# ziadabohalawa/6DoF-Pose-Estimation-and-Defect-Projection

Hardware: AMD Instinct MI355X
Metric: Mrays/s ray-mesh + ICP iters/s, 640x576 vs 100k-tri mesh (higher is better)
Workload: dtype f32 rays / f64 ICP (f32 MFMA filter)

## Files before the change

### 6dof-pose-estimation-and-defect-projection_amd/_lib.py

```python
import ctypes as C
import os
import sys
import threading

import numpy as np

_HERE = os.path.dirname(os.path.abspath(__file__))
LIB_PATH = os.environ.get("PEDP_LIB", os.path.join(_HERE, "libpedp_hip.so"))

HOST, DEVICE = 0, 1
POINT_TO_PLANE, POINT_TO_POINT = 0, 1


class PreprocessParams(C.Structure):
    _fields_ = [("voxel_size", C.c_double), ("plane_distance", C.c_double), ("plane_iterations", C.c_int32),
                ("first_frame", C.c_int32), ("seed", C.c_uint64), ("normal_radius", C.c_double), ("normal_max_nn", C.c_int32),
                ("cluster_min_points", C.c_int32), ("cluster_eps", C.c_double), ("outlier_neighbors", C.c_int32),
                ("flags", C.c_int32), ("outlier_std_ratio", C.c_double), ("average_normal_voxel", C.c_double)]

ALLREDUCE_FN = C.CFUNCTYPE(C.c_int, C.c_void_p, C.c_void_p, C.c_int, C.c_void_p)


class IcpParams(C.Structure):
    _fields_ = [
# ... 82 lines not shown
    "pedp_icp_batched": (C.c_int, [C.c_void_p, C.c_void_p, C.c_void_p, _P(IcpParams), C.c_void_p, C.c_int,
                                   C.c_void_p, C.c_void_p, C.c_void_p]),
    "pedp_icp_batched_ex": (C.c_int, [C.c_void_p, C.c_void_p, C.c_void_p, _P(IcpParams), C.c_void_p, C.c_int,
                                      C.c_void_p, C.c_void_p, C.c_void_p, C.c_void_p]),
    "pedp_nn": (C.c_int, [C.c_void_p, C.c_void_p, C.c_void_p, C.c_void_p, C.c_void_p, C.c_void_p]),
    "pedp_nn_last_sweep_ms": (C.c_int, [C.c_void_p, _P(C.c_float)]),
    "pedp_icp_last_stats": (C.c_int, [C.c_void_p, _P(C.c_int64), _P(C.c_int64), _P(C.c_int64)]),
    "pedp_icp_last_planned_passes": (C.c_int, [C.c_void_p, _P(C.c_int64)]),
    "pedp_icp_last_serial_path": (C.c_int, [C.c_void_p, _P(C.c_int64), _P(C.c_int64)]),
    "pedp_icp_last_head_closed": (C.c_int, [C.c_void_p, _P(C.c_int64), _P(C.c_int64), _P(C.c_int64)]),
    "pedp_icp_last_certified": (C.c_int, [C.c_void_p, _P(C.c_int64), _P(C.c_int64)]),
    "pedp_icp_last_steady": (C.c_int, [C.c_void_p, _P(C.c_int64), _P(C.c_int64)]),
    "pedp_icp_last_steady_followers": (C.c_int, [C.c_void_p, _P(C.c_int64)]),
    "pedp_icp_last_lane_solves": (C.c_int, [C.c_void_p, _P(C.c_int64)]),
    "pedp_debug_nn_bf16": (C.c_int, [C.c_void_p, C.c_void_p, C.c_int64, C.c_void_p, C.c_int64, C.c_void_p]),
    "pedp_debug_solve6": (C.c_int, [C.c_void_p, C.c_int64, C.c_void_p, C.c_void_p, C.c_void_p, C.c_void_p, C.c_void_p, C.c_void_p]),
    "pedp_debug_icp_path": (C.c_int, [C.c_void_p, C.c_void_p, C.c_void_p]),
    "pedp_icp_begin": (C.c_int, [C.c_void_p, C.c_void_p, C.c_void_p, _P(IcpParams), C.c_void_p, C.c_int]),
    "pedp_icp_end": (C.c_int, [C.c_void_p, C.c_void_p, _P(C.c_double), _P(C.c_double), _P(C.c_int32), C.c_void_p, C.c_void_p]),
    "pedp_icp_configure": (C.c_int, [C.c_void_p, C.c_int, C.c_int]),
    "pedp_comm_unique_id": (C.c_int, [C.c_void_p]),
    "pedp_comm_create": (C.c_int, [C.c_void_p, C.c_void_p, C.c_int, C.c_int]),
    "pedp_comm_destroy": (C.c_int, [C.c_void_p]),
    "pedp_comm_size": (C.c_int, [C.c_void_p, _P(C.c_int), _P(C.c_int)]),
    "pedp_comm_allgather": (C.c_int, [C.c_void_p, C.c_void_p, C.c_void_p, C.c_int64]),
    "pedp_comm_allreduce_f64": (C.c_int, [C.c_void_p, C.c_void_p, C.c_int64]),
    "pedp_render": (C.c_int, [C.c_void_p, C.c_void_p, C.c_int64, C.c_void_p, C.c_int64, C.c_void_p, C.c_void_p, C.c_void_p,
                              C.c_void_p, C.c_int, C.c_int, C.c_void_p, C.c_void_p, C.c_int, C.c_void_p, C.c_int, C.c_void_p,
                              C.c_void_p, C.c_void_p, C.c_void_p]),
    "pedp_rasterize": (C.c_int, [C.c_void_p, C.c_void_p, C.c_int, C.c_int64, C.c_void_p, C.c_int64, C.c_int, C.c_int, C.c_int,
# ... 718 lines not shown
    return a.value


def icp_last_lane_solves(ctx):
    a = C.c_int64(0)
    check(load().pedp_icp_last_lane_solves(ctx._h, C.byref(a)), "pedp_icp_last_lane_solves")
    return a.value


ICP_SWITCHES = ("nn_f32", "unfused_finish", "no_visit_plan", "serial_close", "copy_bracket", "head_close", "cert", "steady")
ICP_PATH_FIELDS = ("fused", "dev_result", "copy_bracket", "head", "certify", "plan", "serial_close", "unfused_finish", "exchange",
                   "steady", "steady_from")


class IcpSwitches(C.Structure):
    _fields_ = [(n, C.c_int) for n in ICP_SWITCHES + ("steady_from", "steady_grid", "target_order", "steady_closers", "steady_groups", "lane_solve")]


class IcpPathInputs(C.Structure):
    _fields_ = [("n_source", C.c_int64), ("n_target", C.c_int64), ("radius", C.c_double)] + [
        (n, C.c_int) for n in ("unit_size", "poses", "timed_pass", "exhaustive", "exchange", "batch", "early_exit", "no_steady", "resident")]


class IcpPath(C.Structure):
    _fields_ = [(n, C.c_int) for n in ICP_PATH_FIELDS + ("lane_solve",)]


def icp_path(switches=None, steady_from=5, n_source=1, n_target=1, radius=1.0, unit_size=1, poses=1, timed_pass=-1, lane_solve=None,
             **flags):
    sw = None
    if switches is not None:
# ... 98 lines not shown


def debug_solve6(ctx, A, b):
    A = np.ascontiguousarray(A, np.float64).reshape(-1, 36)
    b = np.ascontiguousarray(b, np.float64).reshape(-1, 6)
    n = len(A)
    if len(b) != n:
        raise ValueError("debug_solve6: A and b differ in their count")
    out = {"x_lanes": np.empty((n, 6), np.float64), "ok_lanes": np.empty(n, np.int32),
           "x_one": np.empty((n, 6), np.float64), "ok_one": np.empty(n, np.int32)}
    check(load().pedp_debug_solve6(ctx._h, n, _ptr(A), _ptr(b), _ptr(out["x_lanes"]), _ptr(out["ok_lanes"]), _ptr(out["x_one"]),
                                   _ptr(out["ok_one"])), "pedp_debug_solve6")
    return out


def icp_begin(ctx, source, target, max_correspondence_distance, init, estimator=POINT_TO_PLANE, max_iteration=30,
              relative_fitness=1e-6, relative_rmse=1e-6, want_trace=False, n_source_global=0, use_comm=False):
    prm = IcpParams()
    prm.max_correspondence_distance = float(max_correspondence_distance)
    prm.estimator = int(estimator)
    prm.max_iteration = int(max_iteration)
    prm.relative_fitness = float(relative_fitness)
    prm.relative_rmse = float(relative_rmse)
    prm.allreduce = C.cast(None, ALLREDUCE_FN)
    prm.allreduce_user = None
    prm.n_source_global = int(n_source_global)
    prm.use_comm = int(bool(use_comm))
    T0 = np.ascontiguousarray(init, dtype=np.float64).reshape(4, 4)
    check(load().pedp_icp_begin(ctx._h, source._h, target._h, C.byref(prm), _ptr(T0), 1 if want_trace else 0), "pedp_icp_begin")
    ctx._icp_pending = (source, target, int(max_iteration), bool(want_trace))
# ... 102 lines not shown
```

### 6dof-pose-estimation-and-defect-projection_amd/csrc/icp/fused_close.h

```cpp
#pragma once
#include "common.h"
#include "solve.h"
#include "solve_lanes.h"

namespace {

constexpr int CH = NN_SB * 16;
constexpr int BK_W = 8;
constexpr int BK_WCAP = BK_W * 64;
constexpr int PSTRIDE = 32;
constexpr int LIVE_CAP = 8192;
constexpr int FIN_THREADS = 1024;

__device__ __forceinline__ void swap_if(bool c, double &x, double &y) {
    const double t = x;
    x = c ? y : x;
    y = c ? t : y;
}
__device__ bool solve6_ldlt_reg(const double *__restrict__ Ain, const double *__restrict__ b, double *__restrict__ x) {
    double A[6][6], y[6];
    int tr[6];
#pragma unroll
    for (int i = 0; i < 6; ++i)
#pragma unroll
// ... 161 lines not shown
    int serial = 0;
    int lane = 0;
    unsigned long long *live_old = nullptr;
    int gen_masks = 0;
};
template <int NT, int LCAP>
struct FinishLds {
    double slice[32][32], pk[32];
    int scan[NT], lst[LCAP];
    int do_rebuild, n_live_s, stopped;
    double t0[16];
};
__device__ __forceinline__ double bcast0(double v) {
    return __hiloint2double(__builtin_amdgcn_readfirstlane(__double2hiint(v)), __builtin_amdgcn_readfirstlane(__double2loint(v)));
}
typedef __attribute__((address_space(1))) unsigned long long g_u64;
typedef __attribute__((address_space(1))) int g_i32;
typedef __attribute__((address_space(1))) unsigned g_u32;
__device__ __forceinline__ double load_sc1(const double *p) {
    return __longlong_as_double((long long)__hip_atomic_load((g_u64 *)(uintptr_t)p, __ATOMIC_RELAXED, __HIP_MEMORY_SCOPE_AGENT));
}
__device__ __forceinline__ int load_sc1(const int32_t *p) {
    return __hip_atomic_load((g_i32 *)(uintptr_t)p, __ATOMIC_RELAXED, __HIP_MEMORY_SCOPE_AGENT);
}
__device__ __forceinline__ void store_sc1(double *p, double v) {
    __hip_atomic_store((g_u64 *)(uintptr_t)p, (unsigned long long)__double_as_longlong(v), __ATOMIC_RELAXED, __HIP_MEMORY_SCOPE_AGENT);
}
template <bool COHERENT>
__device__ __forceinline__ double load_partial(const double *p) {
    return COHERENT ? load_sc1(p) : *p;
}
template <bool COHERENT>
__device__ __forceinline__ unsigned long long load_live(unsigned long long *p) {
    if (COHERENT) return __hip_atomic_fetch_or((g_u64 *)(uintptr_t)p, 0ull, __ATOMIC_RELAXED, __HIP_MEMORY_SCOPE_AGENT);
    return *p;
}

#define PEDP_STAMP_CLOSE(unit, slot) do { if (!HEAD || blockIdx.x == 0) PEDP_STAMP(2, unit, slot); } while (0)
template <int NT, int LCAP, bool COHERENT, int MODE = 0>
__device__ __forceinline__ void icp_finish_body(IcpState *st, const FinishArgs &f, FinishLds<NT, LCAP> &L, const int tid) {
    constexpr bool LOCAL = MODE != 0, HEAD = MODE >= 2;
    static_assert(MODE != 2 || !COHERENT, "the head close reads what the launch before stored");
    static_assert(MODE != 3 || COHERENT, "the close inside a steady launch reads what that launch stored");
    auto uni = [](double v) { return LOCAL ? bcast0(v) : v; };
    const int pass = f.known ? f.k_pass : st->pass, max_iter = LOCAL ? __builtin_amdgcn_readfirstlane(st->max_iter) : st->max_iter;
    const double n_source = uni(st->n_source), rel_fitness = uni(st->rel_fitness), rel_rmse = uni(st->rel_rmse), reachE = uni(st->reachE),
                 margin = uni(st->margin);
    constexpr int PARTS = 32, TPARTS = NT / 32, PPT = PARTS / TPARTS;
    static_assert(NT % 32 == 0 && PARTS % TPARTS == 0, "thread count");
    const bool wide = f.serial == 0;
    if (tid == 0) { L.do_rebuild = 0; L.stopped = 0; }
    if (tid == 0) PEDP_STAMP_CLOSE(0, 0);
    if (tid == 0 && pass == 5) PEDP_STAMP_CLOSE(3, 0);
    const bool early_look = wide && COHERENT && f.n_idle > 0;
    unsigned look0 = 0u, idle_base0 = 0u;
    if (early_look && tid < 64) {
        if (tid < 16) look0 = __hip_atomic_load((g_u32 *)(uintptr_t)(f.idle + 32 * tid), __ATOMIC_RELAXED, __HIP_MEMORY_SCOPE_AGENT);
        idle_base0 = st->idle_base;
    }
    double fit0 = 0.0, rmse0 = 0.0, mu_th0 = 0.0, mu_ta0 = 0.0;
    int n_wide0 = 0;
    if (tid < 16) L.t0[tid] = st->T[tid];
    if (tid == 0) {
        fit0 = st->fitness; rmse0 = st->rmse; mu_th0 = st->mu_theta; mu_ta0 = st->mu_tau;
        if (wide) n_wide0 = st->n_wide;
    }
#if PEDP_ICP_STAMPS
    if (tid == 0 && (!HEAD || blockIdx.x == 0)) { g_icp_stamps[2][1][0] = (long long)__builtin_amdgcn_s_memtime(); g_icp_stamps[2][1][1] = (long long)__builtin_amdgcn_s_memrealtime(); }
#endif
    if (f.phase != 2) {
        const bool listing = !HEAD && (f.known ? f.k_rebuild != 0 : st->rebuild != 0);
        int n_live = f.known ? f.k_n_live : st->n_live;
        bool listed = true;
        if (listing) {
            const int per = (f.n_lw + NT - 1) / NT;
            const int w_lo = tid * per < f.n_lw ? tid * per : f.n_lw, w_hi = w_lo + per < f.n_lw ? w_lo + per : f.n_lw;
            int mine = 0;
            unsigned long long first = 0ull;
            for (int wi = w_lo; wi < w_hi; ++wi) {
                const unsigned long long word = load_live<COHERENT>(&f.live[wi]);
                if (wi == w_lo) first = word;
                mine += __builtin_popcountll(word);
            }
            L.scan[tid] = mine;
            __syncthreads();
            for (int off = 1; off < NT; off <<= 1) {
                const int t = tid >= off ? L.scan[tid - off] : 0;
                __syncthreads();
                L.scan[tid] += t;
                __syncthreads();
            }
            n_live = L.scan[NT - 1];
            listed = n_live <= LCAP;
            int at = L.scan[tid] - mine;
            for (int wi = w_lo; wi < w_hi; ++wi) {
                unsigned long long word = wi == w_lo ? first : load_live<COHERENT>(&f.live[wi]);
                while (word != 0ull) {
                    const int chunk = wi * 64 + __builtin_ctzll(word);
                    word &= word - 1ull;
                    if (listed) L.lst[at] = chunk;
                    as_global(f.live_list)[at] = chunk;
                    ++at;
                }
            }
            __syncthreads();
        }
        const int k = tid & 31;
        const int lper = (n_live + PARTS - 1) / PARTS;
        auto sum_ranges = [&](auto position) {
            if constexpr (PPT == 2) {
                constexpr int BW = 10;
                const int part = tid >> 4, k0 = (tid & 15) * 2, k1 = k0 + 1;
                const bool has1 = k1 < PACKET + (LOCAL ? 3 : 2);
                const int l_lo = part * lper < n_live ? part * lper : n_live, l_hi = l_lo + lper < n_live ? l_lo + lper : n_live;
                double v0 = 0.0, v1 = 0.0;
                for (int q = l_lo; q < l_hi; q += BW) {
                    int at[BW];
                    double x0[BW], x1[BW];
#pragma unroll
                    for (int u = 0; u < BW; ++u) at[u] = position(q + u < l_hi ? q + u : l_hi - 1);
// ... 31 lines not shown
                        double x[BW1];
#pragma unroll
                        for (int u = 0; u < BW1; ++u) at[u] = position(q + u < l_hi ? q + u : l_hi - 1);
#pragma unroll
                        for (int u = 0; u < BW1; ++u) x[u] = load_partial<COHERENT>(&f.partials[(size_t)at[u] * PSTRIDE + k]);
#pragma unroll
                        for (int u = 0; u < BW1; ++u) v = q + u < l_hi ? v + x[u] : v;
                    }
                }
                L.slice[part][k] = v;
            }
        };
        if (!listing) sum_ranges([&](int q) { return q; });
        else if (listed) sum_ranges([&](int q) { return L.lst[q]; });
        else sum_ranges([&](int q) { return load_sc1(&f.live_list[q]); });
        if (tid == 0 && pass == 5) PEDP_STAMP_CLOSE(3, 1);
        if (HEAD) PEDP_RT(pass + 1, 5);
        if (tid == 0) L.n_live_s = n_live;
        __syncthreads();
        if (tid == 0 && pass == 5) PEDP_STAMP_CLOSE(3, 2);
        if (tid < 32) {
            double t = 0.0;
            for (int q = 0; q < PARTS; ++q) t += L.slice[q][tid];
            L.pk[tid] = t;
            if (!HEAD && tid < PACKET) as_global(f.packet)[tid] = t;
        }
        __syncthreads();
        if (HEAD) PEDP_RT(pass + 1, 6);
        if (tid == 0 && f.phase == 1) {
            st->sum_tiles += (long long)L.pk[PACKET];
            st->sum_fb += (long long)L.pk[PACKET + 1];
            st->n_live = L.n_live_s;
        }
        if (tid == 0) {
#if PEDP_ICP_STAMPS
// ... 27 lines not shown
                st->done = -1;
                if (!LOCAL && f.down) *(int *)((char *)f.down + offsetof(IcpState, done)) = -1;
            }
            return;
        }
    }
    if (wide ? tid < 64 : tid == 0) {
        const bool l0 = tid == 0;
        int stop_i = 0, angles_i = 0;
        int solve_i = 0;
        const bool lane_form = wide && f.lane != 0;
        double upd[16], x[6] = {0.0, 0.0, 0.0, 0.0, 0.0, 0.0};
        ident4(upd);
        if (l0) {
            PEDP_STAMP_CLOSE(0, 1);
            if (pass == 5) PEDP_STAMP_CLOSE(3, 3);
            if (COHERENT) { st->ticket_base += (unsigned)f.n_busy; st->idle_base += (unsigned)f.n_idle; }
            if (f.phase == 0) {
                st->sum_tiles += (long long)L.pk[PACKET];
                st->sum_fb += (long long)L.pk[PACKET + 1];
                st->n_live = L.n_live_s;
                if constexpr (LOCAL) {
                    const long long searched = (long long)(L.pk[PACKET + 2] / CERT_PACK);
                    st->sum_searched += searched;
                    st->sum_cert += (long long)(L.pk[PACKET + 2] - (double)searched * CERT_PACK);
                }
            }
            L.do_rebuild = 0;
            const double *pk = L.pk;
            const double K = pk[28];
            double fit = 0.0, rmse = 0.0;
// ... 9 lines not shown
            }
            st->iters = pass;
            if (wide) st->n_wide = n_wide0 + 1;
            if (HEAD) st->n_head = st->n_head + 1;
            bool stop = pass >= max_iter;
            if (pass > 0 && fabs(fit0 - fit) < rel_fitness && fabs(rmse0 - rmse) < rel_rmse) stop = true;
            if (stop) {
                st->done = 1;
                if (!LOCAL && COHERENT && f.down) {
                    L.stopped = 1;
                    asm volatile("s_waitcnt vmcnt(0)" ::: "memory");
                }
                stop_i = 1;
            } else {
                PEDP_STAMP_CLOSE(2, 0);
                if (pass == 5) PEDP_STAMP_CLOSE(3, 4);
                if (K > 0.0) {
                    if (f.estimator == PEDP_POINT_TO_PLANE && lane_form) {
                        solve_i = 1;
                    } else if (f.estimator == PEDP_POINT_TO_PLANE) {
                        double A[36], nb[6];
                        int k = 0;
#pragma unroll
                        for (int u = 0; u < 6; ++u)
#pragma unroll
                            for (int v = u; v < 6; ++v) { A[6 * u + v] = pk[k]; A[6 * v + u] = pk[k]; ++k; }
#pragma unroll
                        for (int u = 0; u < 6; ++u) nb[u] = -pk[21 + u];
                        const bool ok = solve6_ldlt_reg(A, nb, x);
                        PEDP_STAMP_CLOSE(2, 1);
                        if (ok) {
// ... 50 lines not shown
                    if (!lane_form) {
#pragma unroll
                        for (int k = 0; k < 6; ++k) x[k] = bcast0(x[k]);
                    }
                    double s, c;
                    sincos(tid == 0 ? x[0] : (tid == 1 ? x[1] : x[2]), &s, &c);
                    const double sa = __shfl(s, 0, 64), ca = __shfl(c, 0, 64), sb = __shfl(s, 1, 64), cb = __shfl(c, 1, 64),
                                 sc = __shfl(s, 2, 64), cc = __shfl(c, 2, 64);
                    sincos_to_T(sa, ca, sb, cb, sc, cc, x, upd);
                    if (l0) PEDP_STAMP_CLOSE(2, 2);
                } else {
#pragma unroll
                    for (int k = 0; k < 16; ++k) upd[k] = bcast0(upd[k]);
                }
                if (l0) PEDP_STAMP_CLOSE(0, 2);
                if (l0 && pass == 5) PEDP_STAMP_CLOSE(3, 5);
                const int i = (tid >> 2) & 3, j = tid & 3;
                double tn = 0.0, u_ij = 0.0;
#pragma unroll
                for (int k = 0; k < 4; ++k) {
                    const double a = i == 0 ? upd[k] : (i == 1 ? upd[4 + k] : (i == 2 ? upd[8 + k] : upd[12 + k]));
                    const double b = L.t0[4 * k + j];
                    tn += a * b;
                    u_ij = j == k ? a : u_ij;
                }
                if (tid < 16) {
                    st->upd[tid] = u_ij;
                    if (!HEAD) as_global(f.hist)[16 * (pass + 1) + tid] = u_ij;
                    st->T[tid] = tn;
                }
            } else {
                PEDP_STAMP_CLOSE(0, 2);
                if (pass == 5) PEDP_STAMP_CLOSE(3, 5);
                for (int k = 0; k < 16; ++k) { st->upd[k] = upd[k]; if (!HEAD) as_global(f.hist)[16 * (pass + 1) + k] = upd[k]; }
                double Tn[16];
                mat4_mul_dev(upd, L.t0, Tn);
                for (int k = 0; k < 16; ++k) st->T[k] = Tn[k];
            }
            if (l0) {
                double th2 = 0.0, tv[3];
                for (int u = 0; u < 3; ++u) {
                    tv[u] = upd[4 * u + 3];
                    const double cc[3] = {f.bcx, f.bcy, f.bcz};
                    for (int v = 0; v < 3; ++v) {
                        const double dlt = upd[4 * u + v] - (u == v ? 1.0 : 0.0);
                        th2 += dlt * dlt;
                        tv[u] += dlt * cc[v];
                    }
                }
                double mu_th = mu_th0 + sqrt(th2), mu_ta = mu_ta0 + sqrt(tv[0] * tv[0] + tv[1] * tv[1] + tv[2] * tv[2]);
                const double mu = mu_th * reachE + mu_ta;
                if (!(mu < 0.95 * margin)) {
                    L.do_rebuild = 1;
                    mu_th = 0.0;
                    mu_ta = 0.0;
                    st->n_rebuilds += 1;
                }
                st->mu_theta = mu_th;
                st->mu_tau = mu_ta;
                st->rebuild = L.do_rebuild;
                st->pass = pass + 1;
                PEDP_STAMP_CLOSE(2, 3);
                if (pass == 5) PEDP_STAMP_CLOSE(3, 6);
            }
        }
        if (l0) PEDP_STAMP_CLOSE(0, 3);
    }
    __syncthreads();
    if (!HEAD && !f.gen_masks && L.do_rebuild)
        for (int wi = tid; wi < f.n_lw; wi += NT) { as_global(f.live_old)[wi] = load_live<COHERENT>(&f.live[wi]); as_global(f.live)[wi] = 0ull; }
    if (!HEAD && f.gen_masks && f.known && f.k_rebuild)
        for (int wi = tid; wi < f.n_lw; wi += NT) as_global(f.live_old)[wi] = 0ull;
    if (!LOCAL && COHERENT && f.down && L.stopped)
        for (int i = tid; i < (int)(sizeof(IcpState) / sizeof(double)); i += NT) ((double *)f.down)[i] = load_sc1((const double *)st + i);
}

__global__ __launch_bounds__(FIN_THREADS) void icp_finish_kernel(IcpState *st, unsigned long long *live, int32_t *live_list,
                                                         int n_lw, const double *partials, double *packet, int phase, int estimator,
// ... 43 lines not shown
```

### 6dof-pose-estimation-and-defect-projection_amd/csrc/icp/fused_pass.h

```cpp
#pragma once
#include "fused_close.h"
#include "segmented_sweep.h"

namespace {

constexpr int WTL = 1024;
constexpr int L2_WORDS = 8;
constexpr int SW_G = 8;

__device__ __forceinline__ void scan_near_tiles(unsigned long long near, int unit_of_lane, const PassArgs &a, double qx,
                                                double qy, double qz, int lane, double &bd, int &bj) {
    while (near != 0ull) {
        int unit = -1;
#pragma unroll
        for (int g = 0; g < 4; ++g) {
            if (near != 0ull) {
                const int bit = __builtin_ctzll(near);
                near &= near - 1ull;
                const int u = __shfl(unit_of_lane, bit, 64);
                if (g == (lane >> 4)) unit = u;
            }
        }
        const int64_t row = (int64_t)unit * 16 + (lane & 15);
        if (unit >= 0 && row < a.Nt)
// ... 205 lines not shown
                                   __HIP_MEMORY_SCOPE_AGENT);
        return;
    }
#if PEDP_ICP_STAMPS
    if (threadIdx.x == 0 && pass < 32 && blockIdx.x < 512 && blockIdx.y == 0) g_icp_rt[pass][blockIdx.x][0] = rt_entry;
#endif
    PEDP_RT(pass, 1);
    const bool certify = !BATCH && a0.cert != nullptr;
    const float inf = __uint_as_float(0x7F800000u);
    const double dinf = __longlong_as_double(0x7FF0000000000000ll);
    const double dnan = __longlong_as_double(0x7FF8000000000000ll);
    const double ccx_b = BATCH ? st->centroid[0] : 0.0, ccy_b = BATCH ? st->centroid[1] : 0.0, ccz_b = BATCH ? st->centroid[2] : 0.0;
    const float r_search_b = BATCH ? st->r_search : 0.f;
#define PEDP_CC(k, b) (BATCH ? (b) : bcast0(cur.centroid[k]))
    unsigned long long todo = 0ull;
    int todo_base = -64, it = 0;
    if (rebuild && threadIdx.x == 0) {
        double Rs[12];
#pragma unroll
        for (int k = 0; k < 12; ++k) { Rs[k] = PEDP_ST.T[k]; rbs[k] = Rs[k]; }
        double m = 0.0;
#pragma unroll
        for (int u = 0; u < 3; ++u) {
            double row = 0.0;
#pragma unroll
            for (int v = 0; v < 3; ++v) row += fabs(Rs[u] * Rs[v] + Rs[4 + u] * Rs[4 + v] + Rs[8 + u] * Rs[8 + v]);
            m = row > m ? row : m;
        }
        rbs[12] = sqrt(m) * (1.0 + 1e-9);
        rbs[13] = sqrt(PEDP_ST.r2live) * (1.0 + 1e-9);
    }
    __syncthreads();
    for (;;) {
        int tid = threadIdx.x;
        asm volatile("" : "+v"(tid));
        const int lane = tid & 63, wv = __builtin_amdgcn_readfirstlane(tid >> 6);
        const int half = wv >> 2, q4 = wv & 3;
        const int j = lane & 15, g = lane >> 4;
        const int frag = j * 4 + g;
        const unsigned long long lt = (1ull << lane) - 1ull;
        const PEDP_GLOBAL double *Pk_in = as_global(a.Pk) + (size_t)(pass & 1) * a.pp_stride, *Tp_in = as_global(a.Tprev) + (size_t)(pass & 1) * a.pp_stride;
        PEDP_GLOBAL double *Pk_out = as_global(a.Pk) + (size_t)((pass + 1) & 1) * a.pp_stride, *Tp_out = as_global(a.Tprev) + (size_t)((pass + 1) & 1) * a.pp_stride;
        int chunk, unit;
        if (rebuild) {
            bool more = true;
            while (todo == 0ull) {
                todo_base += 64;
                if ((long long)blockIdx.x + (long long)todo_base * (long long)gdim >= (long long)a.n_chunks) { more = false; break; }
                const long long u = (long long)blockIdx.x + (long long)(todo_base + lane) * (long long)gdim;
                bool visit = false, withdraw = false;
                if (u < (long long)a.n_chunks) {
                    double Rs[12];
#pragma unroll
                    for (int k = 0; k < 12; ++k) Rs[k] = rbs[k];
                    const double rscale = rbs[12], reach = rbs[13];
                    const bool was_live = (as_global(PEDP_MASK_OLD)[u >> 6] >> (u & 63)) & 1ull;
#pragma unroll 2
                    for (int sb = 0; sb < 8; ++sb) {
                        const PEDP_GLOBAL double *sp8 = as_global(a.chunk_sph) + (size_t)(8 * u + sb) * 4;
                        const double cx = sp8[0], cy = sp8[1], cz = sp8[2], cr = sp8[3];
                        const double tx = Rs[0] * cx + Rs[1] * cy + Rs[2] * cz + Rs[3], ty = Rs[4] * cx + Rs[5] * cy + Rs[6] * cz + Rs[7],
                                     tz = Rs[8] * cx + Rs[9] * cy + Rs[10] * cz + Rs[11];
                        const double ex = fmax(fmax(a.lo[0] - tx, tx - a.hi[0]), 0.0), ey = fmax(fmax(a.lo[1] - ty, ty - a.hi[1]), 0.0),
                                     ez = fmax(fmax(a.lo[2] - tz, tz - a.hi[2]), 0.0);
                        const double lim = cr * rscale + reach + 1e-9 * (fabs(tx) + fabs(ty) + fabs(tz) + 1.0);
                        visit |= !(cr < 0.0) && !(ex * ex + ey * ey + ez * ez > lim * lim);
                    }
                    withdraw = !visit && (was_live || pass == 0);
                }
                todo = __builtin_amdgcn_ballot_w64(visit);
                unsigned long long wd = __builtin_amdgcn_ballot_w64(withdraw);
                while (wd != 0ull) {
                    const int i = __builtin_ctzll(wd);
                    wd &= wd - 1ull;
                    const int64_t k = ((int64_t)blockIdx.x + (int64_t)(todo_base + i) * gdim) * CH + tid;
                    if (tid < CH && k < a.N) as_global(a.idx_out)[as_global(a.perm)[k]] = -1;
                }
            }
            if (!more) break;
            const int i = __builtin_ctzll(todo);
            todo &= todo - 1ull;
            unit = (int)(blockIdx.x + (unsigned)(todo_base + i) * (unsigned)gdim);
            chunk = unit;
        } else {
            unit = (int)(blockIdx.x + (unsigned)it * (unsigned)gdim);
            ++it;
            if (unit >= n_live) break;
            if (planned && it == 1) { unit = vis[0]; chunk = vis[1]; }
            else chunk = unit == (int)blockIdx.x ? chunk_next : as_global(a.live_list)[unit];
        }
        long long t_chunk0 = 0;
        if (!BATCH && !rebuild) t_chunk0 = (long long)__builtin_amdgcn_s_memtime();
        if (tid == 0) PEDP_STAMP(1, blockIdx.x, 0);
        PEDP_WV(0, __builtin_amdgcn_s_memtime());
        PEDP_WV(9, pass);
        PEDP_WV(10, __builtin_amdgcn_s_memrealtime());
        PEDP_WV(12, ((long long)__builtin_amdgcn_s_getreg(63508) << 32) | (unsigned)__builtin_amdgcn_s_getreg(63492));
        int nsl;
        bool skip = false;
        {
            bool cand = false, near = false, certd = false;
            int pi = -1, jprev = -1;
            float c_new = 0.f;
            double x = 0.0, y = 0.0, z = 0.0, dprev = dnan, d2prev = dnan;
            const int64_t k = (int64_t)chunk * CH + half * 64 + lane;
            const bool valid = k < a.N;
            if (valid) {
                pi = as_global(a.perm)[k];
// ... 542 lines not shown
```

### 6dof-pose-estimation-and-defect-projection_amd/csrc/pedp_icp.hip

```cpp
#include "pedp_internal.h"
#include <atomic>
#include <cmath>
#include <cstddef>
#include <cstdlib>
#include <cstring>
#include <new>

#if defined(__HIP_DEVICE_COMPILE__) && !defined(__gfx950__)
#error "pedp_icp.hip: the fence-free close of a pass rests on gfx950's caches; build with --offload-arch=gfx950 only"
#endif

#include "icp/common.h"
#include "icp/prep.h"
#include "icp/target_order.h"
#include "icp/segmented_sweep.h"
#include "icp/segmented_select.h"
#include "icp/solve.h"
#include "icp/ransac.h"
#include "icp/fused_close.h"
#include "icp/fused_pass.h"
#include "icp/steady_pass.h"

namespace {

// ... 168 lines not shown
}

using IcpSwitches = pedp_icp_switches;
inline const IcpSwitches &icp_switches() {
    static const IcpSwitches sw = [] {
        auto flag = [](const char *name, int unset) { const char *v = getenv(name); return v ? atoi(v) != 0 : unset; };
        auto num = [](const char *name, int unset) { const char *v = getenv(name); return v && *v ? atoi(v) : unset; };
        const char *order = getenv("PEDP_ICP_TARGET_ORDER");
        IcpSwitches s;
        s.nn_f32 = flag("PEDP_NN_F32", 0); s.unfused_finish = flag("PEDP_ICP_UNFUSED_FINISH", 0);
        s.no_visit_plan = flag("PEDP_ICP_NO_VISIT_PLAN", 0); s.serial_close = flag("PEDP_ICP_SERIAL_CLOSE", 0);
        s.copy_bracket = flag("PEDP_ICP_COPY_BRACKET", 0); s.head_close = flag("PEDP_ICP_HEAD_CLOSE", 1);
        s.cert = flag("PEDP_ICP_CERT", 1); s.steady = flag("PEDP_ICP_STEADY", 1);
        s.steady_from = num("PEDP_ICP_STEADY_FROM", 5); s.steady_grid = num("PEDP_ICP_STEADY_GRID", 0);
        s.steady_closers = num("PEDP_ICP_STEADY_CLOSERS", 0); s.steady_groups = num("PEDP_ICP_STEADY_GROUPS", 0);
        s.lane_solve = num("PEDP_ICP_LANE_SOLVE", 1);
        s.target_order = order && !strcmp(order, "hilbert") ? PEDP_TARGET_ORDER_HILBERT
                         : order && !strcmp(order, "compact") ? PEDP_TARGET_ORDER_COMPACT : PEDP_TARGET_ORDER_AUTO;
        return s;
    }();
    return sw;
}

using IcpPath = pedp_icp_path;
using IcpPathInputs = pedp_icp_path_inputs;
inline bool fused_eligible(int qt, bool exhaustive, double r, int64_t Ns, int64_t Nt) {
    return qt == 1 && !exhaustive && r > 0.0 && Ns > 0 && Nt > 0 && (Nt + 1023) / 1024 <= BK_WCAP;
}
inline IcpPath icp_decide_path(const IcpSwitches &sw, const IcpPathInputs &in) {
    IcpPath p{};
    p.fused = fused_eligible(in.unit_size, in.exhaustive, in.radius, in.n_source, in.n_target);
// ... 136 lines not shown
    pa.cert = path.certify ? w.cert : nullptr; pa.cert_stride = (size_t)w.Ns_pad;
    pa.visit = path.plan ? w.visit : nullptr; pa.dur = path.plan ? w.dur : nullptr; pa.visit_cap = w.visit_cap; pa.n_cu = x->num_cus;
}

struct PassLaunch {
    int pass = 0;
    bool steady_launch = false;
    hipEvent_t ev0 = nullptr, ev1 = nullptr;
};

int enqueue_fused_pass(pedp_ctx_t c, const IcpJob &job, const PassLaunch &l) {
    PassArgs pa = job.pa;
    pa.launch = pa.head ? l.pass : 0;
    int64_t g = job.w.n_chunks;
    if (g > 2 * c->num_cus) g = 2 * c->num_cus;
    if (g < 1) g = 1;
    if (pa.head) g += 1;
    if (l.ev0) PEDP_HIP_CHECK(hipEventRecord(l.ev0, c->stream));
    if (l.steady_launch) {
        const int asked = icp_switches().steady_closers;
        const SteadyShape sh = steady_shape(c, job.w.n_chunks);
        double *const follow = job.w.follow_cap > 0 ? job.w.follow : nullptr;
        const int n_closers = asked > 0 ? asked : c->num_cus;
        auto steady = [&](auto kernel, int groups) {
            hipLaunchKernelGGL(kernel, dim3((unsigned)sh.grid), dim3(groups * BK_W * 64), 0, c->stream, job.w.st, pa, follow, job.w.follow_cap, n_closers);
        };
        if (sh.groups == 2) { if (pa.lane_solve) steady(icp_steady_kernel<2, true>, 2); else steady(icp_steady_kernel<2, false>, 2); }
        else { if (pa.lane_solve) steady(icp_steady_kernel<1, true>, 1); else steady(icp_steady_kernel<1, false>, 1); }
    } else {
        const bool batch = job.in.poses > 1;
// ... 927 lines not shown
        hipLaunchKernelGGL(solve6_lanes_debug_kernel, dim3((unsigned)((n + 3) / 4)), dim3(256), 0, c->stream, (const double *)d_A, (const double *)d_b, n, d_x, d_ok);
        hipLaunchKernelGGL(solve6_one_debug_kernel, dim3((unsigned)((n + 3) / 4)), dim3(256), 0, c->stream, (const double *)d_A, (const double *)d_b, n,
                           d_x + 6 * (size_t)n, d_ok + (size_t)n);
        e = hipGetLastError();
    }
    if (e == hipSuccess) e = hipMemcpyAsync(x_lanes, d_x, sizeof(double) * 6 * (size_t)n, hipMemcpyDeviceToHost, c->stream);
    if (e == hipSuccess) e = hipMemcpyAsync(x_one, d_x + 6 * (size_t)n, sizeof(double) * 6 * (size_t)n, hipMemcpyDeviceToHost, c->stream);
    if (e == hipSuccess) e = hipMemcpyAsync(ok_lanes, d_ok, sizeof(int32_t) * (size_t)n, hipMemcpyDeviceToHost, c->stream);
    if (e == hipSuccess) e = hipMemcpyAsync(ok_one, d_ok + (size_t)n, sizeof(int32_t) * (size_t)n, hipMemcpyDeviceToHost, c->stream);
    if (e == hipSuccess) e = hipStreamSynchronize(c->stream);
    (void)hipFree(d_A); (void)hipFree(d_b); (void)hipFree(d_x); (void)hipFree(d_ok);
    PEDP_HIP_CHECK(e);
    return PEDP_OK;
}

int pedp_debug_icp_path(const pedp_icp_switches *switches, const pedp_icp_path_inputs *inputs, pedp_icp_path *path) {
    PEDP_REQUIRE(inputs && path, "pedp_debug_icp_path: null argument");
    *path = icp_decide_path(switches ? *switches : icp_switches(), *inputs);
    return PEDP_OK;
}

int pedp_icp_graph_captures(pedp_ctx_t c, int64_t *captures) {
    PEDP_REQUIRE(c && captures, "pedp_icp_graph_captures: null argument");
    long long n = c->icp_graph_captures;
    for (int k = 0; k < PEDP_MAX_SUB; ++k)
        if (c->sub[k]) n += c->sub[k]->icp_graph_captures;
    *captures = n;
    return PEDP_OK;
}

// ... 70 lines not shown
```

### include/pedp.h

```cpp
#ifndef PEDP_H
#define PEDP_H
#include <stdint.h>
#ifdef __cplusplus
extern "C" {
#endif

typedef enum {
    PEDP_OK = 0,
    PEDP_ERR_BAD_ARG = -1,
    PEDP_ERR_NO_NORMALS = -2,
    PEDP_ERR_HIP = -3,
    PEDP_ERR_ALLOC = -4,
    PEDP_ERR_COLLECTIVE = -5
} pedp_status;

enum { PEDP_HOST = 0, PEDP_DEVICE = 1 };
enum { PEDP_POINT_TO_PLANE = 0, PEDP_POINT_TO_POINT = 1 };

typedef struct pedp_ctx_s *pedp_ctx_t;
typedef struct pedp_mesh_s *pedp_mesh_t;
typedef struct pedp_rayset_s *pedp_rayset_t;
typedef struct pedp_cloud_s *pedp_cloud_t;

int pedp_version(void);
// ... 184 lines not shown
int pedp_icp_last_serial_path(pedp_ctx_t ctx, int64_t *wide_closes, int64_t *bracket);

int pedp_icp_last_head_closed(pedp_ctx_t ctx, int64_t *head_closed, int64_t *rebuilds, int64_t *launches);

int pedp_icp_last_certified(pedp_ctx_t ctx, int64_t *slots, int64_t *searched_slots);

int pedp_icp_last_steady(pedp_ctx_t ctx, int64_t *passes, int64_t *handbacks);

int pedp_icp_last_steady_followers(pedp_ctx_t ctx, int64_t *followers);

int pedp_icp_last_lane_solves(pedp_ctx_t ctx, int64_t *lane_solves);

int pedp_debug_solve6(pedp_ctx_t ctx, int64_t n, const double *A, const double *b, double *x_lanes, int32_t *ok_lanes,
                      double *x_one, int32_t *ok_one);

int pedp_debug_nn_bf16(pedp_ctx_t ctx, const float *src4, int64_t n_src, const float *tgt4, int64_t n_tgt, float *g);

int pedp_debug_target_pack(pedp_ctx_t ctx, pedp_cloud_t cloud, int64_t *rows, int64_t *pad_rows, int32_t *tile_perm,
                           float *tgt4, float *sph16, float *sph64, float *sph1024);

typedef struct pedp_icp_switches {
    int nn_f32, unfused_finish, no_visit_plan, serial_close, copy_bracket;
    int head_close, cert, steady;
    int steady_from;
    int steady_grid;
    int target_order;
    int steady_closers;
    int steady_groups;
    int lane_solve;
} pedp_icp_switches;
typedef struct pedp_icp_path_inputs {
    int64_t n_source, n_target;
    double radius;
    int unit_size;
    int poses;
    int timed_pass;
    int exhaustive;
    int exchange;
    int batch;
    int early_exit;
    int no_steady;
    int resident;
} pedp_icp_path_inputs;
typedef struct pedp_icp_path {
// ... 313 lines not shown
```

Measured before the change: 798.5.

## Parallelize chunk visit test across lanes and use wave-shuffle scan for live list

The rebuild visit test now spreads each chunk's eight bounding spheres over eight lanes, instead of having one lane loop over all eight. The lanes combine their results through a ballot, which shortens the serial per-chunk loop, and withdrawals are spread across waves. The live-list prefix scan moves from a log-step shared-memory scan with many barriers to wave shuffles plus per-wave totals, and the live-word loads are issued earlier in the close. It also adds an optional pass-grid cap knob, a debug entry point, and extra stamps. The trade-off is eight chunks per ballot round instead of 64, which means more rounds.

Measured after the change: 814.1 (median of 6 runs). 1.02x the previous value.

```diff
diff --git a/6dof-pose-estimation-and-defect-projection_amd/_lib.py b/6dof-pose-estimation-and-defect-projection_amd/_lib.py
--- a/6dof-pose-estimation-and-defect-projection_amd/_lib.py
+++ b/6dof-pose-estimation-and-defect-projection_amd/_lib.py
@@ -120,6 +120,7 @@
     "pedp_icp_last_steady_followers": (C.c_int, [C.c_void_p, _P(C.c_int64)]),
     "pedp_icp_last_lane_solves": (C.c_int, [C.c_void_p, _P(C.c_int64)]),
     "pedp_debug_nn_bf16": (C.c_int, [C.c_void_p, C.c_void_p, C.c_int64, C.c_void_p, C.c_int64, C.c_void_p]),
+    "pedp_debug_live_list": (C.c_int, [C.c_void_p, C.c_void_p, C.c_int, C.c_int, C.c_void_p, _P(C.c_int32)]),
     "pedp_debug_solve6": (C.c_int, [C.c_void_p, C.c_int64, C.c_void_p, C.c_void_p, C.c_void_p, C.c_void_p, C.c_void_p, C.c_void_p]),
     "pedp_debug_icp_path": (C.c_int, [C.c_void_p, C.c_void_p, C.c_void_p]),
     "pedp_icp_begin": (C.c_int, [C.c_void_p, C.c_void_p, C.c_void_p, _P(IcpParams), C.c_void_p, C.c_int]),
@@ -868,7 +869,7 @@
 
 
 class IcpSwitches(C.Structure):
-    _fields_ = [(n, C.c_int) for n in ICP_SWITCHES + ("steady_from", "steady_grid", "target_order", "steady_closers", "steady_groups", "lane_solve")]
+    _fields_ = [(n, C.c_int) for n in ICP_SWITCHES + ("steady_from", "steady_grid", "target_order", "steady_closers", "steady_groups", "lane_solve", "pass_grid")]
 
 
 class IcpPathInputs(C.Structure):
@@ -997,6 +998,14 @@
     return out
 
 
+def debug_live_list(ctx, mask_words, threads=512):
+    words = np.ascontiguousarray(mask_words, np.uint64).reshape(-1)
+    lst = np.full(64 * len(words), -1, np.int32)
+    n = C.c_int32(0)
+    check(load().pedp_debug_live_list(ctx._h, _ptr(words), len(words), int(threads), _ptr(lst), C.byref(n)), "pedp_debug_live_list")
+    return int(n.value), lst
+
+
 def icp_begin(ctx, source, target, max_correspondence_distance, init, estimator=POINT_TO_PLANE, max_iteration=30,
               relative_fitness=1e-6, relative_rmse=1e-6, want_trace=False, n_source_global=0, use_comm=False):
     prm = IcpParams()
diff --git a/6dof-pose-estimation-and-defect-projection_amd/csrc/icp/fused_close.h b/6dof-pose-estimation-and-defect-projection_amd/csrc/icp/fused_close.h
--- a/6dof-pose-estimation-and-defect-projection_amd/csrc/icp/fused_close.h
+++ b/6dof-pose-estimation-and-defect-projection_amd/csrc/icp/fused_close.h
@@ -1,5 +1,6 @@
 #pragma once
 #include "common.h"
+#include "live_list.h"
 #include "solve.h"
 #include "solve_lanes.h"
 
@@ -199,9 +200,6 @@
 __device__ __forceinline__ double bcast0(double v) {
     return __hiloint2double(__builtin_amdgcn_readfirstlane(__double2hiint(v)), __builtin_amdgcn_readfirstlane(__double2loint(v)));
 }
-typedef __attribute__((address_space(1))) unsigned long long g_u64;
-typedef __attribute__((address_space(1))) int g_i32;
-typedef __attribute__((address_space(1))) unsigned g_u32;
 __device__ __forceinline__ double load_sc1(const double *p) {
     return __longlong_as_double((long long)__hip_atomic_load((g_u64 *)(uintptr_t)p, __ATOMIC_RELAXED, __HIP_MEMORY_SCOPE_AGENT));
 }
@@ -215,12 +213,10 @@
 __device__ __forceinline__ double load_partial(const double *p) {
     return COHERENT ? load_sc1(p) : *p;
 }
-template <bool COHERENT>
-__device__ __forceinline__ unsigned long long load_live(unsigned long long *p) {
-    if (COHERENT) return __hip_atomic_fetch_or((g_u64 *)(uintptr_t)p, 0ull, __ATOMIC_RELAXED, __HIP_MEMORY_SCOPE_AGENT);
-    return *p;
-}
-
+
+#ifndef PEDP_ICP_STAMP_CLOSE_PASS
+#define PEDP_ICP_STAMP_CLOSE_PASS 5
+#endif
 #define PEDP_STAMP_CLOSE(unit, slot) do { if (!HEAD || blockIdx.x == 0) PEDP_STAMP(2, unit, slot); } while (0)
 template <int NT, int LCAP, bool COHERENT, int MODE = 0>
 __device__ __forceinline__ void icp_finish_body(IcpState *st, const FinishArgs &f, FinishLds<NT, LCAP> &L, const int tid) {
@@ -236,13 +232,16 @@
     const bool wide = f.serial == 0;
     if (tid == 0) { L.do_rebuild = 0; L.stopped = 0; }
     if (tid == 0) PEDP_STAMP_CLOSE(0, 0);
-    if (tid == 0 && pass == 5) PEDP_STAMP_CLOSE(3, 0);
+    if (tid == 0 && pass == PEDP_ICP_STAMP_CLOSE_PASS) PEDP_STAMP_CLOSE(3, 0);
     const bool early_look = wide && COHERENT && f.n_idle > 0;
     unsigned look0 = 0u, idle_base0 = 0u;
     if (early_look && tid < 64) {
         if (tid < 16) look0 = __hip_atomic_load((g_u32 *)(uintptr_t)(f.idle + 32 * tid), __ATOMIC_RELAXED, __HIP_MEMORY_SCOPE_AGENT);
         idle_base0 = st->idle_base;
     }
+    const bool listing = f.phase != 2 && !HEAD && (f.known ? f.k_rebuild != 0 : st->rebuild != 0);
+    LiveWords lw = {0, 0, 0, 0ull};
+    if (listing) lw = live_words_load<NT, COHERENT>(f.live, f.n_lw, tid);
     double fit0 = 0.0, rmse0 = 0.0, mu_th0 = 0.0, mu_ta0 = 0.0;
     int n_wide0 = 0;
     if (tid < 16) L.t0[tid] = st->T[tid];
@@ -254,41 +253,12 @@
     if (tid == 0 && (!HEAD || blockIdx.x == 0)) { g_icp_stamps[2][1][0] = (long long)__builtin_amdgcn_s_memtime(); g_icp_stamps[2][1][1] = (long long)__builtin_amdgcn_s_memrealtime(); }
 #endif
     if (f.phase != 2) {
-        const bool listing = !HEAD && (f.known ? f.k_rebuild != 0 : st->rebuild != 0);
         int n_live = f.known ? f.k_n_live : st->n_live;
         bool listed = true;
         if (listing) {
-            const int per = (f.n_lw + NT - 1) / NT;
-            const int w_lo = tid * per < f.n_lw ? tid * per : f.n_lw, w_hi = w_lo + per < f.n_lw ? w_lo + per : f.n_lw;
-            int mine = 0;
-            unsigned long long first = 0ull;
-            for (int wi = w_lo; wi < w_hi; ++wi) {
-                const unsigned long long word = load_live<COHERENT>(&f.live[wi]);
-                if (wi == w_lo) first = word;
-                mine += __builtin_popcountll(word);
-            }
-            L.scan[tid] = mine;
-            __syncthreads();
-            for (int off = 1; off < NT; off <<= 1) {
-                const int t = tid >= off ? L.scan[tid - off] : 0;
-                __syncthreads();
-                L.scan[tid] += t;
-                __syncthreads();
-            }
-            n_live = L.scan[NT - 1];
+            n_live = live_list_build<NT, LCAP, COHERENT>(lw, f.live, f.live_list, L.lst, L.scan, tid);
             listed = n_live <= LCAP;
-            int at = L.scan[tid] - mine;
-            for (int wi = w_lo; wi < w_hi; ++wi) {
-                unsigned long long word = wi == w_lo ? first : load_live<COHERENT>(&f.live[wi]);
-                while (word != 0ull) {
-                    const int chunk = wi * 64 + __builtin_ctzll(word);
-                    word &= word - 1ull;
-                    if (listed) L.lst[at] = chunk;
-                    as_global(f.live_list)[at] = chunk;
-                    ++at;
-                }
-            }
-            __syncthreads();
+            if (tid == 0 && pass == PEDP_ICP_STAMP_CLOSE_PASS) PEDP_STAMP_CLOSE(3, 7);
         }
         const int k = tid & 31;
         const int lper = (n_live + PARTS - 1) / PARTS;
@@ -350,11 +320,11 @@
         if (!listing) sum_ranges([&](int q) { return q; });
         else if (listed) sum_ranges([&](int q) { return L.lst[q]; });
         else sum_ranges([&](int q) { return load_sc1(&f.live_list[q]); });
-        if (tid == 0 && pass == 5) PEDP_STAMP_CLOSE(3, 1);
+        if (tid == 0 && pass == PEDP_ICP_STAMP_CLOSE_PASS) PEDP_STAMP_CLOSE(3, 1);
         if (HEAD) PEDP_RT(pass + 1, 5);
         if (tid == 0) L.n_live_s = n_live;
         __syncthreads();
-        if (tid == 0 && pass == 5) PEDP_STAMP_CLOSE(3, 2);
+        if (tid == 0 && pass == PEDP_ICP_STAMP_CLOSE_PASS) PEDP_STAMP_CLOSE(3, 2);
         if (tid < 32) {
             double t = 0.0;
             for (int q = 0; q < PARTS; ++q) t += L.slice[q][tid];
@@ -412,7 +382,7 @@
         ident4(upd);
         if (l0) {
             PEDP_STAMP_CLOSE(0, 1);
-            if (pass == 5) PEDP_STAMP_CLOSE(3, 3);
+            if (pass == PEDP_ICP_STAMP_CLOSE_PASS) PEDP_STAMP_CLOSE(3, 3);
             if (COHERENT) { st->ticket_base += (unsigned)f.n_busy; st->idle_base += (unsigned)f.n_idle; }
             if (f.phase == 0) {
                 st->sum_tiles += (long long)L.pk[PACKET];
@@ -452,7 +422,7 @@
                 stop_i = 1;
             } else {
                 PEDP_STAMP_CLOSE(2, 0);
-                if (pass == 5) PEDP_STAMP_CLOSE(3, 4);
+                if (pass == PEDP_ICP_STAMP_CLOSE_PASS) PEDP_STAMP_CLOSE(3, 4);
                 if (K > 0.0) {
                     if (f.estimator == PEDP_POINT_TO_PLANE && lane_form) {
                         solve_i = 1;
@@ -533,7 +503,7 @@
                     for (int k = 0; k < 16; ++k) upd[k] = bcast0(upd[k]);
                 }
                 if (l0) PEDP_STAMP_CLOSE(0, 2);
-                if (l0 && pass == 5) PEDP_STAMP_CLOSE(3, 5);
+                if (l0 && pass == PEDP_ICP_STAMP_CLOSE_PASS) PEDP_STAMP_CLOSE(3, 5);
                 const int i = (tid >> 2) & 3, j = tid & 3;
                 double tn = 0.0, u_ij = 0.0;
 #pragma unroll
@@ -550,7 +520,7 @@
                 }
             } else {
                 PEDP_STAMP_CLOSE(0, 2);
-                if (pass == 5) PEDP_STAMP_CLOSE(3, 5);
+                if (pass == PEDP_ICP_STAMP_CLOSE_PASS) PEDP_STAMP_CLOSE(3, 5);
                 for (int k = 0; k < 16; ++k) { st->upd[k] = upd[k]; if (!HEAD) as_global(f.hist)[16 * (pass + 1) + k] = upd[k]; }
                 double Tn[16];
                 mat4_mul_dev(upd, L.t0, Tn);
@@ -580,7 +550,7 @@
                 st->rebuild = L.do_rebuild;
                 st->pass = pass + 1;
                 PEDP_STAMP_CLOSE(2, 3);
-                if (pass == 5) PEDP_STAMP_CLOSE(3, 6);
+                if (pass == PEDP_ICP_STAMP_CLOSE_PASS) PEDP_STAMP_CLOSE(3, 6);
             }
         }
         if (l0) PEDP_STAMP_CLOSE(0, 3);
diff --git a/6dof-pose-estimation-and-defect-projection_amd/csrc/icp/fused_pass.h b/6dof-pose-estimation-and-defect-projection_amd/csrc/icp/fused_pass.h
--- a/6dof-pose-estimation-and-defect-projection_amd/csrc/icp/fused_pass.h
+++ b/6dof-pose-estimation-and-defect-projection_amd/csrc/icp/fused_pass.h
@@ -243,7 +243,10 @@
     const float r_search_b = BATCH ? st->r_search : 0.f;
 #define PEDP_CC(k, b) (BATCH ? (b) : bcast0(cur.centroid[k]))
     unsigned long long todo = 0ull;
-    int todo_base = -64, it = 0;
+    int todo_base = -8, it = 0;
+#if PEDP_ICP_STAMPS
+    bool rt_first = true;
+#endif
     if (rebuild && threadIdx.x == 0) {
         double Rs[12];
 #pragma unroll
@@ -274,40 +277,53 @@
         if (rebuild) {
             bool more = true;
             while (todo == 0ull) {
-                todo_base += 64;
+                todo_base += 8;
                 if ((long long)blockIdx.x + (long long)todo_base * (long long)gdim >= (long long)a.n_chunks) { more = false; break; }
-                const long long u = (long long)blockIdx.x + (long long)(todo_base + lane) * (long long)gdim;
-                bool visit = false, withdraw = false;
-                if (u < (long long)a.n_chunks) {
+                const long long u = (long long)blockIdx.x + (long long)(todo_base + (lane >> 3)) * (long long)gdim;
+                const bool inside = u < (long long)a.n_chunks;
+                const long long uc = inside ? u : 0;
+                typedef double v2d __attribute__((ext_vector_type(2)));
+                const PEDP_GLOBAL v2d *sp8 = (const PEDP_GLOBAL v2d *)(uintptr_t)(a.chunk_sph + (size_t)(8 * uc + (lane & 7)) * 4);
+                const v2d sxy = sp8[0], szr = sp8[1];
+                const unsigned long long old_word = as_global(PEDP_MASK_OLD)[uc >> 6];
+                bool near_box;
+                {
                     double Rs[12];
 #pragma unroll
                     for (int k = 0; k < 12; ++k) Rs[k] = rbs[k];
                     const double rscale = rbs[12], reach = rbs[13];
-                    const bool was_live = (as_global(PEDP_MASK_OLD)[u >> 6] >> (u & 63)) & 1ull;
-#pragma unroll 2
-                    for (int sb = 0; sb < 8; ++sb) {
-                        const PEDP_GLOBAL double *sp8 = as_global(a.chunk_sph) + (size_t)(8 * u + sb) * 4;
-                        const double cx = sp8[0], cy = sp8[1], cz = sp8[2], cr = sp8[3];
-                        const double tx = Rs[0] * cx + Rs[1] * cy + Rs[2] * cz + Rs[3], ty = Rs[4] * cx + Rs[5] * cy + Rs[6] * cz + Rs[7],
-                                     tz = Rs[8] * cx + Rs[9] * cy + Rs[10] * cz + Rs[11];
-                        const double ex = fmax(fmax(a.lo[0] - tx, tx - a.hi[0]), 0.0), ey = fmax(fmax(a.lo[1] - ty, ty - a.hi[1]), 0.0),
-                                     ez = fmax(fmax(a.lo[2] - tz, tz - a.hi[2]), 0.0);
-                        const double lim = cr * rscale + reach + 1e-9 * (fabs(tx) + fabs(ty) + fabs(tz) + 1.0);
-                        visit |= !(cr < 0.0) && !(ex * ex + ey * ey + ez * ez > lim * lim);
-                    }
-                    withdraw = !visit && (was_live || pass == 0);
-                }
-                todo = __builtin_amdgcn_ballot_w64(visit);
-                unsigned long long wd = __builtin_amdgcn_ballot_w64(withdraw);
-                while (wd != 0ull) {
-                    const int i = __builtin_ctzll(wd);
-                    wd &= wd - 1ull;
-                    const int64_t k = ((int64_t)blockIdx.x + (int64_t)(todo_base + i) * gdim) * CH + tid;
-                    if (tid < CH && k < a.N) as_global(a.idx_out)[as_global(a.perm)[k]] = -1;
+                    const double cx = sxy[0], cy = sxy[1], cz = szr[0], cr = szr[1];
+                    const double tx = Rs[0] * cx + Rs[1] * cy + Rs[2] * cz + Rs[3], ty = Rs[4] * cx + Rs[5] * cy + Rs[6] * cz + Rs[7],
+                                 tz = Rs[8] * cx + Rs[9] * cy + Rs[10] * cz + Rs[11];
+                    const double ex = fmax(fmax(a.lo[0] - tx, tx - a.hi[0]), 0.0), ey = fmax(fmax(a.lo[1] - ty, ty - a.hi[1]), 0.0),
+                                 ez = fmax(fmax(a.lo[2] - tz, tz - a.hi[2]), 0.0);
+                    const double lim = cr * rscale + reach + 1e-9 * (fabs(tx) + fabs(ty) + fabs(tz) + 1.0);
+                    near_box = inside && !(ex * ex + ey * ey + ez * ez > lim * lim) && !(cr < 0.0);
+                }
+                const unsigned long long nb = __builtin_amdgcn_ballot_w64(near_box);
+                const bool visit = ((nb >> (lane & 56)) & 0xFFull) != 0ull;
+                const bool was_live = (old_word >> (uc & 63)) & 1ull;
+                const bool withdraw = inside && !visit && (was_live || pass == 0);
+                todo = __builtin_amdgcn_ballot_w64(visit && (lane & 7) == 0);
+                const unsigned long long wd = __builtin_amdgcn_ballot_w64(withdraw && (lane & 7) == 0);
+                if (wd != 0ull) {
+                    int64_t kq[2];
+                    int pq[2];
+#pragma unroll
+                    for (int q = 0; q < 2; ++q) {
+                        unsigned long long rest = wd;
+                        for (int s = 0; s < 4 * q + (wv >> 1); ++s) rest &= rest - 1ull;
+                        kq[q] = rest != 0ull ? ((int64_t)blockIdx.x + (int64_t)(todo_base + (__builtin_ctzll(rest) >> 3)) * gdim) * CH + (tid & (CH - 1))
+                                             : a.N;
+                        pq[q] = kq[q] < a.N ? as_global(a.perm)[kq[q]] : 0;
+                    }
+#pragma unroll
+                    for (int q = 0; q < 2; ++q)
+                        if (kq[q] < a.N) as_global(a.idx_out)[pq[q]] = -1;
                 }
             }
             if (!more) break;
-            const int i = __builtin_ctzll(todo);
+            const int i = __builtin_ctzll(todo) >> 3;
             todo &= todo - 1ull;
             unit = (int)(blockIdx.x + (unsigned)(todo_base + i) * (unsigned)gdim);
             chunk = unit;
@@ -321,6 +337,10 @@
         long long t_chunk0 = 0;
         if (!BATCH && !rebuild) t_chunk0 = (long long)__builtin_amdgcn_s_memtime();
         if (tid == 0) PEDP_STAMP(1, blockIdx.x, 0);
+#if PEDP_ICP_STAMPS
+        if (!close_here && rt_first) PEDP_RT(pass, 5);
+        rt_first = false;
+#endif
         PEDP_WV(0, __builtin_amdgcn_s_memtime());
         PEDP_WV(9, pass);
         PEDP_WV(10, __builtin_amdgcn_s_memrealtime());
diff --git a/6dof-pose-estimation-and-defect-projection_amd/csrc/icp/live_list.h b/6dof-pose-estimation-and-defect-projection_amd/csrc/icp/live_list.h
--- /dev/null
+++ b/6dof-pose-estimation-and-defect-projection_amd/csrc/icp/live_list.h
@@ -0,0 +1,78 @@
+#pragma once
+#include "common.h"
+
+namespace {
+
+typedef __attribute__((address_space(1))) unsigned long long g_u64;
+typedef __attribute__((address_space(1))) int g_i32;
+typedef __attribute__((address_space(1))) unsigned g_u32;
+template <bool COHERENT>
+__device__ __forceinline__ unsigned long long load_live(unsigned long long *p) {
+    if (COHERENT) return __hip_atomic_fetch_or((g_u64 *)(uintptr_t)p, 0ull, __ATOMIC_RELAXED, __HIP_MEMORY_SCOPE_AGENT);
+    return *p;
+}
+
+struct LiveWords {
+    int w_lo, w_hi, mine;
+    unsigned long long first;
+};
+template <int NT, bool COHERENT>
+__device__ __forceinline__ LiveWords live_words_load(unsigned long long *live, int n_lw, int tid) {
+    const int per = (n_lw + NT - 1) / NT;
+    LiveWords w;
+    w.w_lo = tid * per < n_lw ? tid * per : n_lw;
+    w.w_hi = w.w_lo + per < n_lw ? w.w_lo + per : n_lw;
+    w.mine = 0;
+    w.first = 0ull;
+    for (int wi = w.w_lo; wi < w.w_hi; ++wi) {
+        const unsigned long long word = load_live<COHERENT>(&live[wi]);
+        if (wi == w.w_lo) w.first = word;
+        w.mine += __builtin_popcountll(word);
+    }
+    return w;
+}
+template <int NT, int LCAP, bool COHERENT>
+__device__ __forceinline__ int live_list_build(const LiveWords &w, unsigned long long *live, int32_t *live_list, int *lst, int *wave_tot,
+                                               int tid) {
+    static_assert(NT % 64 == 0, "whole waves");
+    const int lane = tid & 63, wave = tid >> 6;
+    int incl = w.mine;
+#pragma unroll
+    for (int off = 1; off < 64; off <<= 1) {
+        const int t = __shfl_up(incl, off, 64);
+        incl += lane >= off ? t : 0;
+    }
+    if (lane == 63) wave_tot[wave] = incl;
+    __syncthreads();
+    int before = 0, n_live = 0;
+#pragma unroll
+    for (int q = 0; q < NT / 64; ++q) {
+        const int t = wave_tot[q];
+        before += q < wave ? t : 0;
+        n_live += t;
+    }
+    const bool listed = n_live <= LCAP;
+    int at = before + incl - w.mine;
+    for (int wi = w.w_lo; wi < w.w_hi; ++wi) {
+        unsigned long long word = wi == w.w_lo ? w.first : load_live<COHERENT>(&live[wi]);
+        while (word != 0ull) {
+            const int chunk = wi * 64 + __builtin_ctzll(word);
+            word &= word - 1ull;
+            if (listed) lst[at] = chunk;
+            as_global(live_list)[at] = chunk;
+            ++at;
+        }
+    }
+    __syncthreads();
+    return n_live;
+}
+
+template <int NT, int LCAP, bool COHERENT>
+__global__ __launch_bounds__(NT) void live_list_debug_kernel(unsigned long long *live, int n_lw, int32_t *list_out, int32_t *n_live_out) {
+    __shared__ int lst[LCAP], wave_tot[NT / 64];
+    const LiveWords w = live_words_load<NT, COHERENT>(live, n_lw, threadIdx.x);
+    const int n_live = live_list_build<NT, LCAP, COHERENT>(w, live, list_out, lst, wave_tot, threadIdx.x);
+    if (threadIdx.x == 0) *n_live_out = n_live;
+}
+
+}
diff --git a/6dof-pose-estimation-and-defect-projection_amd/csrc/pedp_icp.hip b/6dof-pose-estimation-and-defect-projection_amd/csrc/pedp_icp.hip
--- a/6dof-pose-estimation-and-defect-projection_amd/csrc/pedp_icp.hip
+++ b/6dof-pose-estimation-and-defect-projection_amd/csrc/pedp_icp.hip
@@ -206,7 +206,7 @@
         s.cert = flag("PEDP_ICP_CERT", 1); s.steady = flag("PEDP_ICP_STEADY", 1);
         s.steady_from = num("PEDP_ICP_STEADY_FROM", 5); s.steady_grid = num("PEDP_ICP_STEADY_GRID", 0);
         s.steady_closers = num("PEDP_ICP_STEADY_CLOSERS", 0); s.steady_groups = num("PEDP_ICP_STEADY_GROUPS", 0);
-        s.lane_solve = num("PEDP_ICP_LANE_SOLVE", 1);
+        s.lane_solve = num("PEDP_ICP_LANE_SOLVE", 1); s.pass_grid = num("PEDP_ICP_PASS_GRID", 0);
         s.target_order = order && !strcmp(order, "hilbert") ? PEDP_TARGET_ORDER_HILBERT
                          : order && !strcmp(order, "compact") ? PEDP_TARGET_ORDER_COMPACT : PEDP_TARGET_ORDER_AUTO;
         return s;
@@ -373,6 +373,7 @@
     pa.launch = pa.head ? l.pass : 0;
     int64_t g = job.w.n_chunks;
     if (g > 2 * c->num_cus) g = 2 * c->num_cus;
+    if (!l.steady_launch && icp_switches().pass_grid > 0 && g > icp_switches().pass_grid) g = icp_switches().pass_grid;
     if (g < 1) g = 1;
     if (pa.head) g += 1;
     if (l.ev0) PEDP_HIP_CHECK(hipEventRecord(l.ev0, c->stream));
@@ -1330,6 +1331,30 @@
     return PEDP_OK;
 }
 
+int pedp_debug_live_list(pedp_ctx_t c, const unsigned long long *mask_words, int n_lw, int threads, int32_t *list_out, int32_t *n_live_out) {
+    PEDP_REQUIRE(c && mask_words && list_out && n_live_out && n_lw > 0 && n_lw <= (1 << 20) && (threads == BK_W * 64 || threads == FIN_THREADS),
+                 "pedp_debug_live_list: null argument, a word count outside 1 .. 2^20, or a thread count other than 512 and 1024");
+    PEDP_HIP_CHECK(hipSetDevice(c->device));
+    unsigned long long *d_m = nullptr;
+    int32_t *d_l = nullptr;
+    const size_t cap = 64 * (size_t)n_lw;
+    hipError_t e = hipMalloc((void **)&d_m, sizeof(unsigned long long) * (size_t)n_lw);
+    if (e == hipSuccess) e = hipMalloc((void **)&d_l, sizeof(int32_t) * (cap + 1));
+    if (e == hipSuccess) e = hipMemcpyAsync(d_m, mask_words, sizeof(unsigned long long) * (size_t)n_lw, hipMemcpyHostToDevice, c->stream);
+    if (e == hipSuccess) e = hipMemcpyAsync(d_l, list_out, sizeof(int32_t) * cap, hipMemcpyHostToDevice, c->stream);
+    if (e == hipSuccess) {
+        if (threads == BK_W * 64) hipLaunchKernelGGL((live_list_debug_kernel<BK_W * 64, 2048, true>), dim3(1), dim3(BK_W * 64), 0, c->stream, d_m, n_lw, d_l, d_l + cap);
+        else hipLaunchKernelGGL((live_list_debug_kernel<FIN_THREADS, LIVE_CAP, false>), dim3(1), dim3(FIN_THREADS), 0, c->stream, d_m, n_lw, d_l, d_l + cap);
+        e = hipGetLastError();
+    }
+    if (e == hipSuccess) e = hipMemcpyAsync(list_out, d_l, sizeof(int32_t) * cap, hipMemcpyDeviceToHost, c->stream);
+    if (e == hipSuccess) e = hipMemcpyAsync(n_live_out, d_l + cap, sizeof(int32_t), hipMemcpyDeviceToHost, c->stream);
+    if (e == hipSuccess) e = hipStreamSynchronize(c->stream);
+    (void)hipFree(d_m); (void)hipFree(d_l);
+    PEDP_HIP_CHECK(e);
+    return PEDP_OK;
+}
+
 int pedp_debug_icp_path(const pedp_icp_switches *switches, const pedp_icp_path_inputs *inputs, pedp_icp_path *path) {
     PEDP_REQUIRE(inputs && path, "pedp_debug_icp_path: null argument");
     *path = icp_decide_path(switches ? *switches : icp_switches(), *inputs);
diff --git a/include/pedp.h b/include/pedp.h
--- a/include/pedp.h
+++ b/include/pedp.h
@@ -222,6 +222,8 @@
 int pedp_debug_solve6(pedp_ctx_t ctx, int64_t n, const double *A, const double *b, double *x_lanes, int32_t *ok_lanes,
                       double *x_one, int32_t *ok_one);
 
+int pedp_debug_live_list(pedp_ctx_t ctx, const unsigned long long *mask_words, int n_lw, int threads, int32_t *list_out, int32_t *n_live_out);
+
 int pedp_debug_nn_bf16(pedp_ctx_t ctx, const float *src4, int64_t n_src, const float *tgt4, int64_t n_tgt, float *g);
 
 int pedp_debug_target_pack(pedp_ctx_t ctx, pedp_cloud_t cloud, int64_t *rows, int64_t *pad_rows, int32_t *tile_perm,
@@ -236,6 +238,7 @@
     int steady_closers;
     int steady_groups;
     int lane_solve;
+    int pass_grid;
 } pedp_icp_switches;
 typedef struct pedp_icp_path_inputs {
     int64_t n_source, n_target;
```
